# wavey-ai/mel-spec

Hardware: AMD Instinct MI355X
Metric: mel frames/sec/GPU (Whisper 400/160/80 @16 kHz); realtime x vs CPU ref (higher is better)
Workload: dtype f32

## Files before the change

mel_spec_amd/csrc/device_fft.hpp:

```cpp
#pragma once

#if defined(__HIPCC__)
#define MS_DEV __device__ __forceinline__
#ifndef MS_SCHED_LOADS_FIRST
#define MS_SCHED_LOADS_FIRST 0x108
#endif
#define MS_HD __host__ __device__ __forceinline__
#else
#define MS_DEV inline
#define MS_HD inline
#endif
#define MS_RESTRICT __restrict__

namespace melspec {

template <class T>
struct cpx {
    T re, im;
};
using cf = cpx<float>;
using cd = cpx<double>;
struct alignas(8) f2 {
    float x, y;
};
struct alignas(16) f4 {
    float x, y, z, w;
};
struct alignas(16) d2 {
    double x, y;
};

MS_DEV f2 ld2(const float *p) {
#if defined(__HIPCC__)
    typedef float v2f __attribute__((ext_vector_type(2)));
    const v2f v = *reinterpret_cast<const v2f *>(p);
    return f2{v.x, v.y};
#else
    return f2{p[0], p[1]};
#endif
}
MS_DEV f2 ld2_single(const float *p) {
#if defined(__HIPCC__)
    typedef float v2f __attribute__((ext_vector_type(2)));
    typedef const volatile __attribute__((address_space(3))) v2f *lds_ptr;
    const v2f v = *(lds_ptr)(p);
    return f2{v.x, v.y};
#else
    return f2{p[0], p[1]};
#endif
}
MS_DEV f4 ld4(const float *p) {
#if defined(__HIPCC__)
    typedef float v4f __attribute__((ext_vector_type(4)));
    const v4f v = *reinterpret_cast<const v4f *>(p);
    return f4{v.x, v.y, v.z, v.w};
#else
    return f4{p[0], p[1], p[2], p[3]};
#endif
}

template <class T> struct PairOf;
template <> struct PairOf<float> { using type = f2; };
template <> struct PairOf<double> { using type = d2; };
template <class T> MS_DEV cpx<T> ldc(const T *p) {
    const typename PairOf<T>::type v = *reinterpret_cast<const typename PairOf<T>::type *>(p);
    return {v.x, v.y};
}
template <class T> MS_DEV void stc(T *p, cpx<T> v) {
    *reinterpret_cast<typename PairOf<T>::type *>(p) = typename PairOf<T>::type{v.re, v.im};
}

MS_HD float f32_mul_rn(float a, float b) {
#if defined(__HIP_DEVICE_COMPILE__)
    float p = a * b;
    asm("" : "+v"(p));
    return p;
#else
    volatile float p = a * b;
    return p;
#endif
}
MS_DEV int fresh_lane_value(int v) {
#if defined(__HIP_DEVICE_COMPILE__)
    asm volatile("" : "+v"(v));
#endif
    return v;
}
MS_HD float f32_div_rn(float a, float b) {
#if defined(__HIP_DEVICE_COMPILE__)
    return __fdiv_rn(a, b);
#else
    return a / b;
#endif
}
template <class T> MS_DEV cpx<T> operator+(cpx<T> a, cpx<T> b) { return {a.re + b.re, a.im + b.im}; }
template <class T> MS_DEV cpx<T> operator-(cpx<T> a, cpx<T> b) { return {a.re - b.re, a.im - b.im}; }
template <class T> MS_DEV cpx<T> cmul(cpx<T> a, cpx<T> b) { return {a.re * b.re - a.im * b.im, a.re * b.im + a.im * b.re}; }
template <class T> MS_DEV cpx<T> mul_neg_i(cpx<T> a) { return {a.im, -a.re}; }

template <class T>
MS_DEV void bf2(cpx<T> &a, cpx<T> &b) {
    const cpx<T> t = a - b;
    a = a + b;
    b = t;
}

template <class T>
MS_DEV void bf4(cpx<T> &x0, cpx<T> &x1, cpx<T> &x2, cpx<T> &x3) {
    const cpx<T> s0 = x0 + x2, s1 = x0 - x2, s2 = x1 + x3, s3 = mul_neg_i(x1 - x3);
    x0 = s0 + s2;
    x1 = s1 + s3;
    x2 = s0 - s2;
    x3 = s1 - s3;
}

template <class T>
MS_DEV void bf5(cpx<T> &x0, cpx<T> &x1, cpx<T> &x2, cpx<T> &x3, cpx<T> &x4) {
    constexpr T c1 = static_cast<T>(0.30901699437494742410);
    constexpr T c2 = static_cast<T>(-0.80901699437494742410);
    constexpr T s1 = static_cast<T>(0.95105651629515357212);
    constexpr T s2 = static_cast<T>(0.58778525229247312917);
    const cpx<T> t1 = x1 + x4, t2 = x2 + x3, t3 = x1 - x4, t4 = x2 - x3;
    const cpx<T> m1 = {x0.re + c1 * t1.re + c2 * t2.re, x0.im + c1 * t1.im + c2 * t2.im};
    const cpx<T> m2 = {x0.re + c2 * t1.re + c1 * t2.re, x0.im + c2 * t1.im + c1 * t2.im};
    const cpx<T> u1 = {s1 * t3.re + s2 * t4.re, s1 * t3.im + s2 * t4.im};
    const cpx<T> u2 = {s2 * t3.re - s1 * t4.re, s2 * t3.im - s1 * t4.im};
    x0 = x0 + t1 + t2;
    x1 = {m1.re + u1.im, m1.im - u1.re};
    x4 = {m1.re - u1.im, m1.im + u1.re};
    x2 = {m2.re + u2.im, m2.im - u2.re};
    x3 = {m2.re - u2.im, m2.im + u2.re};
}

template <class T>
MS_DEV void fft10(cpx<T> (&x)[10]) {
    cpx<T> a[2][5];
#pragma unroll
    for (int n1 = 0; n1 < 2; ++n1)
#pragma unroll
        for (int n2 = 0; n2 < 5; ++n2) a[n1][n2] = x[(5 * n1 + 2 * n2) % 10];
#pragma unroll
    for (int n2 = 0; n2 < 5; ++n2) bf2(a[0][n2], a[1][n2]);
#pragma unroll
    for (int k1 = 0; k1 < 2; ++k1) bf5(a[k1][0], a[k1][1], a[k1][2], a[k1][3], a[k1][4]);
#pragma unroll
    for (int k1 = 0; k1 < 2; ++k1)
#pragma unroll
        for (int k2 = 0; k2 < 5; ++k2) x[(5 * k1 + 6 * k2) % 10] = a[k1][k2];
}

template <class T>
MS_DEV void fft20(cpx<T> (&x)[20]) {
    cpx<T> a[4][5];
#pragma unroll
    for (int n1 = 0; n1 < 4; ++n1)
#pragma unroll
        for (int n2 = 0; n2 < 5; ++n2) a[n1][n2] = x[(5 * n1 + 4 * n2) % 20];
#pragma unroll
    for (int n2 = 0; n2 < 5; ++n2) bf4(a[0][n2], a[1][n2], a[2][n2], a[3][n2]);
#pragma unroll
    for (int k1 = 0; k1 < 4; ++k1) bf5(a[k1][0], a[k1][1], a[k1][2], a[k1][3], a[k1][4]);
#pragma unroll
    for (int k1 = 0; k1 < 4; ++k1)
#pragma unroll
        for (int k2 = 0; k2 < 5; ++k2) x[(5 * k1 + 16 * k2) % 20] = a[k1][k2];
}

template <class T>
MS_DEV void fft8(cpx<T> (&x)[8]) {
    constexpr T r = static_cast<T>(0.70710678118654752440);
#pragma unroll
    for (int n2 = 0; n2 < 4; ++n2) bf2(x[n2], x[n2 + 4]);
    x[5] = {r * (x[5].re + x[5].im), r * (x[5].im - x[5].re)};
    x[6] = mul_neg_i(x[6]);
    x[7] = {r * (x[7].im - x[7].re), -r * (x[7].re + x[7].im)};
    bf4(x[0], x[1], x[2], x[3]);
    bf4(x[4], x[5], x[6], x[7]);
    const cpx<T> y0 = x[0], y1 = x[4], y2 = x[1], y3 = x[5], y4 = x[2], y5 = x[6], y6 = x[3], y7 = x[7];
    x[0] = y0; x[1] = y1; x[2] = y2; x[3] = y3; x[4] = y4; x[5] = y5; x[6] = y6; x[7] = y7;
}

template <class T>
MS_DEV void fft16(cpx<T> (&x)[16]) {
    constexpr T c1 = static_cast<T>(0.92387953251128675613), s1 = static_cast<T>(0.38268343236508977173);
    constexpr T r = static_cast<T>(0.70710678118654752440);
#pragma unroll
    for (int n2 = 0; n2 < 4; ++n2) bf4(x[n2], x[n2 + 4], x[n2 + 8], x[n2 + 12]);
    x[5] = cmul(x[5], cpx<T>{c1, -s1});
    x[6] = cpx<T>{r * (x[6].re + x[6].im), r * (x[6].im - x[6].re)};
    x[7] = cmul(x[7], cpx<T>{s1, -c1});
    x[9] = cpx<T>{r * (x[9].re + x[9].im), r * (x[9].im - x[9].re)};
    x[10] = mul_neg_i(x[10]);
    x[11] = cpx<T>{r * (x[11].im - x[11].re), -r * (x[11].re + x[11].im)};
    x[13] = cmul(x[13], cpx<T>{s1, -c1});
    x[14] = cpx<T>{r * (x[14].im - x[14].re), -r * (x[14].re + x[14].im)};
    x[15] = cmul(x[15], cpx<T>{-c1, s1});
#pragma unroll
    for (int k1 = 0; k1 < 4; ++k1) bf4(x[4 * k1], x[4 * k1 + 1], x[4 * k1 + 2], x[4 * k1 + 3]);
    cpx<T> y[16];
#pragma unroll
    for (int k1 = 0; k1 < 4; ++k1)
#pragma unroll
        for (int k2 = 0; k2 < 4; ++k2) y[k1 + 4 * k2] = x[4 * k1 + k2];
#pragma unroll
    for (int i = 0; i < 16; ++i) x[i] = y[i];
}

}
```

mel_spec_amd/csrc/fast_tables.hpp:

```cpp
#pragma once
#include <cstdint>
#include <cstring>
#include <vector>

#include "tables.hpp"
#include "whisper_fast.hpp"

namespace melspec {

struct FastTables {
    std::vector<float> blob;
    MelSlots slots{};
    int n_mels = 0;
    int nnz = 0;
    bool interval = false;
};

inline bool build_interval_mel(const std::vector<double> &dense, int n_mels, int bins, int bin_limit,
                               std::vector<float> &b, MelSlots &slots, int lanes = 12, double scale = 0.25,
                               int starts_off = FastBlob::kMelStart, int max_slots = kMaxSlots) {
    const int real = lanes - 1;
    std::vector<int> idx(bin_limit, -1);
    for (int k = 0; k < bin_limit; ++k) {
        int lo = -1, hi = -1;
        for (int m = 0; m < n_mels; ++m)
            if (dense[static_cast<size_t>(m) * bins + k] != 0.0) { if (lo < 0) lo = m; hi = m; }
        if (lo < 0) continue;
        if (hi - lo > 1) return false;
        if (hi != lo) { idx[k] = hi; continue; }
        const double *row = &dense[static_cast<size_t>(lo) * bins];
        int peak = 0;
        for (int q = 1; q < bin_limit; ++q) if (row[q] > row[peak]) peak = q;
        idx[k] = (k <= peak) ? lo : lo + 1;
    }
    int last = -1;
    for (int k = 0; k < bin_limit; ++k) {
        if (idx[k] < 0) continue;
        if (idx[k] < last) return false;
        last = idx[k];
    }
    const int n_int = n_mels + 1;
    std::vector<int> first(n_int, 0), cnt(n_int, 0);
    for (int k = 0; k < bin_limit; ++k) {
        if (idx[k] < 0) continue;
        if (cnt[idx[k]] == 0) first[idx[k]] = k;
        else if (first[idx[k]] + cnt[idx[k]] != k) return false;
        ++cnt[idx[k]];
    }
    const int n_slots = (n_int + real - 1) / real;
    if (n_slots > max_slots || n_slots > kSlotCap) return false;
    slots = MelSlots{};
    slots.n_slots = n_slots;
    for (int s = 0; s < n_slots; ++s) {
        int L = 0;
        for (int j = 0; j < lanes; ++j) {
            const int i = s * real + j;
            if (i < n_int && cnt[i] > L) L = cnt[i];
        }
        slots.len[s] = L;
        slots.woff[s] = static_cast<int>(b.size());
        b.resize(b.size() + static_cast<size_t>(L) * lanes * 2, 0.0f);
        for (int j = 0; j < lanes; ++j) {
            const int i = s * real + j;
            int st = 0;
            if (i < n_int && cnt[i] > 0) {
                st = first[i];
                if (st + L > bin_limit) st = bin_limit - L;
                for (int r = 0; r < L; ++r) {
                    const int k = st + r;
                    if (idx[k] != i) continue;
                    const double rise = i < n_mels ? dense[static_cast<size_t>(i) * bins + k] : 0.0;
                    const double fall = i >= 1 ? dense[static_cast<size_t>(i - 1) * bins + k] : 0.0;
                    b[slots.woff[s] + (r * lanes + j) * 2] = static_cast<float>(scale * rise);
                    b[slots.woff[s] + (r * lanes + j) * 2 + 1] = static_cast<float>(scale * fall);
                }
            }
            std::memcpy(&b[starts_off + s * lanes + j], &st, sizeof(int));
        }
    }
    return true;
}

inline bool build_fast_tables(const std::vector<double> &dense, int n_mels, FastTables &out, bool want_interval = false) {
    constexpr int N = 400, M = 200;
    const int n_slots = (n_mels + kMelJobs - 1) / kMelJobs;
    if (n_mels < 1 || n_slots > kMaxSlots) return false;
    std::vector<float> &b = out.blob;
    b.assign(FastBlob::kMelW, 0.0f);
    const std::vector<double> win = hann_window(N);
    for (int t = 0; t < 10; ++t)
        for (int n1 = 0; n1 < 20; ++n1)
            for (int c = 0; c < 2; ++c) b[FastBlob::kWin + t * FastBlob::kWinStride + 2 * n1 + c] = static_cast<float>(win[20 * n1 + 2 * t + c]);
    for (int t = 0; t < 10; ++t)
        for (int k1 = 0; k1 < 20; ++k1) {
            const double a = -2.0 * kPi * ((t * k1) % M) / M;
            b[FastBlob::kTw1 + t * FastBlob::kTw1Stride + 2 * k1] = static_cast<float>(std::cos(a));
            b[FastBlob::kTw1 + t * FastBlob::kTw1Stride + 2 * k1 + 1] = static_cast<float>(std::sin(a));
        }
    for (int n2 = 0; n2 < 10; ++n2) {
        const double a = -2.0 * kPi * n2 / 10.0;
        b[FastBlob::kMod + 2 * n2] = static_cast<float>(std::cos(a));
        b[FastBlob::kMod + 2 * n2 + 1] = static_cast<float>(std::sin(a));
    }
    for (int j = 0; j < kMelJobs; ++j)
        for (int q = 0; q < 10; ++q) {
            const double a = -2.0 * kPi * (j + 20 * q) / N;
            b[FastBlob::kTw2 + j * 20 + 2 * q] = static_cast<float>(std::cos(a));
            b[FastBlob::kTw2 + j * 20 + 2 * q + 1] = static_cast<float>(std::sin(a));
        }
    const int bins = N / 2 + 1;
    const BandedFilterbank fb = band_filterbank(dense, n_mels, bins, M);
    out.nnz = fb.nnz;
    out.n_mels = n_mels;
    out.interval = false;
    if (want_interval && build_interval_mel(dense, n_mels, bins, M, b, out.slots)) {
        out.interval = true;
        while (b.size() % 4) b.push_back(0.0f);
        return true;
    }
    b.resize(FastBlob::kMelW);
    out.slots = MelSlots{};
    out.slots.n_slots = n_slots;
    for (int i = 0; i < n_slots; ++i) {
        int L = 0;
        for (int j = 0; j < kMelJobs; ++j) {
            const int m = i * kMelJobs + j;
            if (m < n_mels && fb.len[m] > L) L = fb.len[m];
        }
        out.slots.len[i] = L;
        out.slots.woff[i] = static_cast<int>(b.size());
        b.resize(b.size() + static_cast<size_t>(L) * kMelJobs, 0.0f);
        for (int j = 0; j < kMelJobs; ++j) {
            const int m = i * kMelJobs + j;
            int st = 0;
            if (m < n_mels && fb.len[m] > 0) {
                st = fb.start[m];
                if (st + L > M) st = M - L;
                for (int r = 0; r < L; ++r)
                    b[out.slots.woff[i] + r * kMelJobs + j] =
                        static_cast<float>(dense[static_cast<size_t>(m) * bins + st + r]);
            }
            std::memcpy(&b[FastBlob::kMelStart + i * kMelJobs + j], &st, sizeof(int));
        }
    }
    while (b.size() % 4) b.push_back(0.0f);
    return true;
}

inline bool build_fast_tables(double sr, int n_mels, FastTables &out, bool want_interval = false) {
    return build_fast_tables(mel_filterbank(sr, 400, n_mels, -1.0, -1.0, false, true), n_mels, out, want_interval);
}

}

#include "whisper_wave_f64.hpp"
#include "whisper_six.hpp"
#include "whisper_six64.hpp"

namespace melspec {

inline bool build_six_tables(const std::vector<double> &dense, int n_mels, FastTables &out, int max_slots = kSixMaxSlots) {
    constexpr int N = 400, M = 200;
    if (n_mels < 1 || n_mels > kSixOwn * max_slots - 1) return false;
    std::vector<float> &b = out.blob;
    b.assign((SixBlob::kMelStart + max_slots * kSixLanes + 3) & ~3, 0.0f);
    const std::vector<double> win = hann_window(N);
    for (int t = 0; t < 10; ++t)
        for (int n1 = 0; n1 < 20; ++n1)
            for (int c = 0; c < 2; ++c) b[SixBlob::kWin + t * SixBlob::kWinStride + 2 * n1 + c] = static_cast<float>(win[20 * n1 + 2 * t + c]);
    for (int t = 0; t < 10; ++t)
        for (int k1 = 0; k1 < 20; ++k1) {
            const double a = -2.0 * kPi * ((t * k1) % M) / M;
            b[SixBlob::kTw1 + t * SixBlob::kTw1Stride + 2 * k1] = static_cast<float>(std::cos(a));
            b[SixBlob::kTw1 + t * SixBlob::kTw1Stride + 2 * k1 + 1] = static_cast<float>(std::sin(a));
        }
    for (int j = 0; j < kSixLanes; ++j)
        for (int s = 0; s < 11; ++s) {
            int k = j + 20 * s;
            if (j == 0) k = s < 6 ? 20 * s : 10 + 20 * (s - 6);
            const double a = -2.0 * kPi * k / N;
            b[SixBlob::kTw2 + j * SixBlob::kTw2Stride + 2 * s] = static_cast<float>(std::cos(a));
            b[SixBlob::kTw2 + j * SixBlob::kTw2Stride + 2 * s + 1] = static_cast<float>(std::sin(a));
        }
    const int bins = N / 2 + 1;
    out.n_mels = n_mels;
    out.nnz = 0;
    out.interval = build_interval_mel(dense, n_mels, bins, M, b, out.slots, kSixLanes, 0.25, SixBlob::kMelStart, max_slots);
    while (b.size() % 4) b.push_back(0.0f);
    return out.interval;
}

inline bool build_six_tables(double sr, int n_mels, FastTables &out) {
    return build_six_tables(mel_filterbank(sr, 400, n_mels, -1.0, -1.0, false, true), n_mels, out);
}

struct PreciseTables {
    std::vector<uint32_t> blob;
    int mel_off_words = 0;
};

inline bool build_precise_tables(const FastTables &ft, PreciseTables &out, bool power_split) {
    if (!ft.interval) return false;
    constexpr int N = 400, M = 200;
    std::vector<double> t(PreciseBlob::kCount, 0.0);
    const std::vector<double> win = hann_window(N);
    for (int i = 0; i < N; ++i) t[PreciseBlob::kWin + i] = win[i];
    for (int tt = 0; tt < 10; ++tt)
        for (int k1 = 0; k1 < 20; ++k1) {
            const double a = -2.0 * kPi * ((tt * k1) % M) / M;
            t[PreciseBlob::kTw1 + tt * PreciseBlob::kTw1Stride + 2 * k1] = std::cos(a);
            t[PreciseBlob::kTw1 + tt * PreciseBlob::kTw1Stride + 2 * k1 + 1] = std::sin(a);
        }
    for (int n2 = 0; n2 < 10; ++n2) {
        const double a = -2.0 * kPi * n2 / 10.0;
        t[PreciseBlob::kMod + 2 * n2] = std::cos(a);
        t[PreciseBlob::kMod + 2 * n2 + 1] = std::sin(a);
    }
    for (int j = 0; j < kMelJobs; ++j)
        for (int q = 0; q < 10; ++q) {
            const double a = -2.0 * kPi * (j + 20 * q) / N;
            t[PreciseBlob::kTw2 + j * PreciseBlob::kTw2Stride + 2 * q] = power_split ? 2.0 * std::sin(a) : std::cos(a);
            t[PreciseBlob::kTw2 + j * PreciseBlob::kTw2Stride + 2 * q + 1] = power_split ? 4.0 * std::cos(a) : std::sin(a);
        }
    const size_t t_words = t.size() * 2;
    const size_t mel_floats = ft.blob.size() - FastBlob::kMelStart;
    out.mel_off_words = static_cast<int>(t_words);
    out.blob.assign(t_words + mel_floats, 0u);
    std::memcpy(out.blob.data(), t.data(), t.size() * sizeof(double));
    std::memcpy(out.blob.data() + t_words, ft.blob.data() + FastBlob::kMelStart, mel_floats * sizeof(float));
    while (out.blob.size() % 4) out.blob.push_back(0u);
    return true;
}

struct Six64Tables {
    std::vector<uint32_t> blob;
    int mel_off_words = 0;
};

inline bool build_six64_tables(const FastTables &ft6, Six64Tables &out) {
    if (!ft6.interval) return false;
    constexpr int N = 400, M = 200;
    std::vector<double> t(Six64Blob::kCount, 0.0);
    const std::vector<double> win = hann_window(N);
    for (int tt = 0; tt < 10; ++tt)
        for (int n1 = 0; n1 < 20; ++n1)
            for (int c = 0; c < 2; ++c) t[Six64Blob::kWin + tt * Six64Blob::kWinStride + 2 * n1 + c] = win[20 * n1 + 2 * tt + c];
    for (int tt = 0; tt < 10; ++tt)
        for (int k1 = 0; k1 < 20; ++k1) {
            const double a = -2.0 * kPi * ((tt * k1) % M) / M;
            t[Six64Blob::kTw1 + tt * Six64Blob::kTw1Stride + 2 * k1] = std::cos(a);
            t[Six64Blob::kTw1 + tt * Six64Blob::kTw1Stride + 2 * k1 + 1] = std::sin(a);
        }
    for (int j = 0; j < kSixLanes; ++j)
        for (int s = 0; s < 11; ++s) {
            int k = j + 20 * s;
            if (j == 0) k = s < 6 ? 20 * s : 10 + 20 * (s - 6);
            const double a = -2.0 * kPi * k / N;
            t[Six64Blob::kTw2 + j * Six64Blob::kTw2Stride + 2 * s] = 2.0 * std::sin(a);
            t[Six64Blob::kTw2 + j * Six64Blob::kTw2Stride + 2 * s + 1] = 4.0 * std::cos(a);
        }
    const size_t t_words = t.size() * 2;
    const size_t mel_floats = ft6.blob.size() - SixBlob::kMelStart;
    out.mel_off_words = static_cast<int>(t_words);
    out.blob.assign(t_words + mel_floats, 0u);
    std::memcpy(out.blob.data(), t.data(), t.size() * sizeof(double));
    std::memcpy(out.blob.data() + t_words, ft6.blob.data() + SixBlob::kMelStart, mel_floats * sizeof(float));
    while (out.blob.size() % 4) out.blob.push_back(0u);
    return true;
}

}
```

mel_spec_amd/csrc/whisper_six.hpp:

```cpp
#pragma once
#include "whisper_wave.hpp"

namespace melspec {

constexpr int kSixFrames = 6;
constexpr int kSixLanes = 10;
constexpr int kSixOwn = 9;
#ifndef MELSPEC_SIX_WAVES
#define MELSPEC_SIX_WAVES 16
#endif
constexpr int kSixWaves = MELSPEC_SIX_WAVES;
constexpr int kSixMaxSlots = 9;
constexpr int kSixWideSlots = 15;
constexpr int kSixWideWaves = 12;

struct SixBlob {
    static constexpr int kWinStride = 44;
    static constexpr int kWin = 0;
    static constexpr int kTw1 = 10 * kWinStride;
    static constexpr int kTw1Stride = 44;
    static constexpr int kTw2Stride = 28;
    static constexpr int kTw2 = kTw1 + 10 * kTw1Stride;
    static constexpr int kMelStart = kTw2 + 10 * kTw2Stride;
    static constexpr int kMelW = (kMelStart + kSixMaxSlots * kSixLanes + 3) & ~3;
};

struct SixLayout {
    static constexpr int kXRow = 20;
    static constexpr int kXStride = 404;
    static constexpr int kPStride = 213;
    static constexpr int kPmaxOff = 1280;
    static constexpr int kPmaxStride = 12;
    static constexpr int slice_floats() { return kSixFrames * kXStride; }
    MS_HD static constexpr int row_pos(int k1) {
        constexpr int t[20] = {14, 1, 13, 4, 16, 3, 17, 11, 6, 8, 19, 9, 7, 15, 18, 5, 2, 12, 0, 10};
        return t[k1];
    }
    MS_HD static void row_offsets(int j, int &uoff, int &voff) {
        uoff = 0; voff = 0;
        for (int k = 0; k < kSixLanes; ++k)
            if (k == j) { uoff = row_pos(k) * kXRow; voff = row_pos(k == 0 ? 10 : 20 - k) * kXRow; }
    }
};

template <int MELS, int... L>
struct LensSixStatic {
    static constexpr bool kStatic = true;
    static constexpr int kSlots = sizeof...(L);
    static constexpr int kMels = MELS;
    MS_HD static constexpr int len(int i) {
        constexpr int t[sizeof...(L)] = {L...};
        return t[i];
    }
    MS_HD static constexpr int woff(int i) {
        constexpr int t[sizeof...(L)] = {L...};
        int s = 0;
        for (int k = 0; k < i; ++k) s += t[k];
        return SixBlob::kMelW + 2 * kSixLanes * s;
    }
};
using LensSix80 = LensSixStatic<80, 1, 1, 1, 2, 2, 3, 4, 6, 7>;
template <int MELS, int... L>
struct LensSixWideStatic {
    static constexpr bool kStatic = true;
    static constexpr int kSlots = sizeof...(L);
    static constexpr int kMels = MELS;
    static constexpr int kMelW = (SixBlob::kMelStart + kSixWideSlots * kSixLanes + 3) & ~3;
    MS_HD static constexpr int len(int i) {
        constexpr int t[sizeof...(L)] = {L...};
        return t[i];
    }
    MS_HD static constexpr int woff(int i) {
        constexpr int t[sizeof...(L)] = {L...};
        int s = 0;
        for (int k = 0; k < i; ++k) s += t[k];
        return kMelW + 2 * kSixLanes * s;
    }
};
using LensSix128 = LensSixWideStatic<128, 1, 1, 1, 1, 1, 1, 1, 2, 2, 2, 3, 3, 4, 5, 5>;
using LensSix64 = LensSixStatic<64, 2, 2, 2, 3, 4, 6, 10, 10>;
using LensSix40 = LensSixStatic<40, 2, 3, 5, 11, 14>;

template <class In>
MS_DEV void six_phase1(int fl, int t, bool active, int hop, const float *blob, const In *gsrc ,
                       float *slice) {
    if (!active) return;
    const In *s = gsrc + fl * hop + 2 * t;
    cf x[20];
    const float *w = blob + SixBlob::kWin + t * SixBlob::kWinStride;
    f2 sv[20];
#pragma unroll
    for (int n1 = 0; n1 < 20; ++n1) sv[n1] = load2_unaligned(s + 20 * n1);
#if defined(__HIP_DEVICE_COMPILE__)
    __builtin_amdgcn_sched_barrier(MS_SCHED_LOADS_FIRST);
#endif
#pragma unroll
    for (int n1 = 0; n1 < 20; n1 += 2) {
        const f4 wv = ld4(w + 2 * n1);
        x[n1] = {sv[n1].x * wv.x, sv[n1].y * wv.y};
        x[n1 + 1] = {sv[n1 + 1].x * wv.z, sv[n1 + 1].y * wv.w};
    }
    fft20(x);
    const float *tw = blob + SixBlob::kTw1 + t * SixBlob::kTw1Stride;
    float *xo = slice + fl * SixLayout::kXStride + 2 * t;
    *reinterpret_cast<f2 *>(xo + SixLayout::row_pos(0) * SixLayout::kXRow) = f2{x[0].re, x[0].im};
#pragma unroll
    for (int k1 = 1; k1 < 20; ++k1) {
        const f2 wv = *reinterpret_cast<const f2 *>(tw + 2 * k1);
        const cf y = cmul(x[k1], cf{wv.x, wv.y});
        *reinterpret_cast<f2 *>(xo + SixLayout::row_pos(k1) * SixLayout::kXRow) = f2{y.re, y.im};
    }
}

MS_DEV void six_phase2(int fl, int j, bool active, const float *blob, float *slice, int uoff, int voff) {
    if (!active) return;
    const float *ua = slice + fl * SixLayout::kXStride + uoff;
    const float *va = slice + fl * SixLayout::kXStride + voff;
    cf u[10], v[10];
#pragma unroll
    for (int i = 0; i < 5; ++i) {
        const f4 a = *reinterpret_cast<const f4 *>(ua + 4 * i);
        const f4 b = *reinterpret_cast<const f4 *>(va + 4 * i);
        u[2 * i] = {a.x, a.y};
        u[2 * i + 1] = {a.z, a.w};
        v[2 * i] = {b.x, b.y};
        v[2 * i + 1] = {b.z, b.w};
    }
    fft10(u);
    fft10(v);
    const bool lane0 = j == 0;
    const int koff = lane0 ? -110 : j;
    const float *tw = blob + SixBlob::kTw2 + j * SixBlob::kTw2Stride;
    float *p = slice + fl * SixLayout::kPStride;
    auto pair = [&](cf zk, cf zm, cf W, float &pk, float &pm) {
        const cf S = {zk.re + zm.re, zk.im - zm.im};
        const cf D = {zk.re - zm.re, zk.im + zm.im};
        const cf wd = cmul(W, D);
        const float ar = S.re + wd.im, ai = S.im - wd.re;
        const float br = S.re - wd.im, bi = S.im + wd.re;
        pk = ar * ar + ai * ai;
        pm = br * br + bi * bi;
    };
#pragma unroll
    for (int s = 0; s < 10; s += 2) {
        const f4 w2 = *reinterpret_cast<const f4 *>(tw + 2 * s);
        float pk[2], pm[2];
#pragma unroll
        for (int h = 0; h < 2; ++h) {
            const int ss = s + h;
            cf zk, zm;
            if (ss < 6) {
                const cf own = u[(10 - ss) % 10];
                zk = u[ss];
                zm = {lane0 ? own.re : v[9 - ss].re, lane0 ? own.im : v[9 - ss].im};
            } else {
                zk = {lane0 ? v[ss - 6].re : u[ss].re, lane0 ? v[ss - 6].im : u[ss].im};
                zm = {lane0 ? v[15 - ss].re : v[9 - ss].re, lane0 ? v[15 - ss].im : v[9 - ss].im};
            }
            const cf W = h == 0 ? cf{w2.x, w2.y} : cf{w2.z, w2.w};
            pair(zk, zm, W, pk[h], pm[h]);
        }
        const int k = (s < 6 ? j : koff) + 20 * s;
        p[k] = pk[0];
        p[k + 20] = pk[1];
        p[200 - k] = pm[0];
        p[180 - k] = pm[1];
    }
    if (lane0) {
        const f2 w2 = *reinterpret_cast<const f2 *>(tw + 20);
        float pk, pm;
        pair(v[4], v[5], cf{w2.x, w2.y}, pk, pm);
        p[90] = pk;
        p[110] = pm;
    }
}

template <int NSLOTS, class Lens>
MS_DEV void six_phase3_sums(int fl, int j, bool active, const MelSlots &ms, const float *blob, const float *slice,
                            const int (&st)[NSLOTS], float (&rise)[NSLOTS], float (&fprev)[NSLOTS]) {
    const float *p = slice + (active ? fl : 0) * SixLayout::kPStride;
#pragma unroll
    for (int i = 0; i < NSLOTS; ++i) {
        float ar = 0.0f, af = 0.0f;
        if (Lens::kStatic) {
            if (i < Lens::kSlots) {
                const float *pp = p + st[i];
                const float *w = blob + Lens::woff(i < Lens::kSlots ? i : 0) + 2 * j;
#pragma unroll
                for (int r = 0; r < Lens::len(i < Lens::kSlots ? i : 0); ++r) {
                    const f2 wv = ld2_single(w + 2 * kSixLanes * r);
                    const float pv = pp[r];
                    if (r == 0) { ar = wv.x * pv; af = wv.y * pv; }
                    else { ar += wv.x * pv; af += wv.y * pv; }
#if defined(__HIP_DEVICE_COMPILE__)
                    if (Lens::len(i < Lens::kSlots ? i : 0) > 7 && r % 5 == 4 && r + 1 < Lens::len(i < Lens::kSlots ? i : 0))
                        __builtin_amdgcn_sched_barrier(0);
#endif
                }
            }
        } else if (i < ms.n_slots) {
            const float *pp = p + st[i];
            const float *w = blob + ms.woff[i] + 2 * j;
            interval_bins_runtime<2 * kSixLanes>(pp, w, ms.len[i], ar, af);
        }
        rise[i] = ar;
        fprev[i] = af;
    }
}

MS_DEV int six_bits(float v) { return __builtin_bit_cast(int, v); }
MS_DEV float six_float(int v) { return __builtin_bit_cast(float, v); }
MS_DEV int six_imax(int a, int b) { return a > b ? a : b; }
MS_DEV int six_imin(int a, int b) { return a < b ? a : b; }
template <int NSLOTS>
MS_DEV void six_phase3_finish(int fl, int j, bool active, int n_mels, const float (&rise)[NSLOTS],
                              const float (&fnext)[NSLOTS] , float *slice, float (&vals)[NSLOTS]) {
    if (!active) return;
    int mx = 0;
#pragma unroll
    for (int i = 0; i < NSLOTS; ++i) {
        const float e = rise[i] + fnext[i];
        const float v = __builtin_fmaxf(fast_log2(e) * 0.30102999566398120f + 16.0f, 6.0f);
        vals[i] = v;
        if (j < kSixOwn && j + kSixOwn * i < n_mels) mx = six_imax(mx, six_bits(v));
    }
    reinterpret_cast<int *>(slice)[SixLayout::kPmaxOff + fl * SixLayout::kPmaxStride + j] = mx;
}

struct alignas(16) SixI4 { int x, y, z, w; };
struct alignas(8) SixI2 { int x, y; };
MS_DEV float six_out(int c) { return six_float(c) * 0.25f - 3.0f; }
template <int NSLOTS, bool LAYOUT = false, bool GUARD = false, bool KEYS = false, class Out = float>
MS_DEV bool six_phase4(int fl, int j, bool store, bool valid, int n_mels, const float *slice, const float (&vals)[NSLOTS],
                       Out *out_tile, long long row_w, int *kmin = nullptr, int *kmax = nullptr) {
    if (!LAYOUT) { valid = true; row_w = 0; }
    if (!store || j >= kSixOwn) return false;
    int lo = 0;
    if (valid) {
        const int *pm = reinterpret_cast<const int *>(slice) + SixLayout::kPmaxOff + fl * SixLayout::kPmaxStride;
        const SixI4 a = *reinterpret_cast<const SixI4 *>(pm), b = *reinterpret_cast<const SixI4 *>(pm + 4);
        const SixI2 c = *reinterpret_cast<const SixI2 *>(pm + 8);
        const int m0 = six_imax(six_imax(a.x, a.y), six_imax(a.z, a.w));
        const int m1 = six_imax(six_imax(b.x, b.y), six_imax(b.z, b.w));
        lo = six_bits(six_float(six_imax(six_imax(m0, m1), six_imax(c.x, c.y))) - 8.0f);
    }
    Out *o = row_w ? out_tile + static_cast<long long>(j) * row_w + fl : out_tile + static_cast<long long>(fl) * n_mels + j;
    const long long step = row_w ? kSixOwn * row_w : kSixOwn;
    int cmin = 0x7f000000, cmax = 0;
#pragma unroll
    for (int i = 0; i < NSLOTS; ++i) {
        const int m = j + kSixOwn * i;
        if (m < n_mels) {
            const int c = valid ? six_imax(six_bits(vals[i]), lo) : 0x41400000;
            o[i * step] = static_cast<Out>(six_out(c));
            if (GUARD || KEYS) cmin = six_imin(cmin, c);
            if (KEYS) cmax = six_imax(cmax, c);
        }
    }
    if (KEYS) { *kmin = cmin; *kmax = cmax; }
    return GUARD && valid && six_float(cmin) < six_float(lo) + kGuardBand;
}

}
```

Baseline: 3.404 billion.

## Special-case DC/Nyquist bins, FMA-based radix-5 butterfly, and unconditional mel log

Adds a float-specialised radix-5 butterfly that forms the conjugate-pair outputs with FMAs, deriving x4 and x3 from x1 and x2 as 2*m - x. Reworks the real-FFT post-processing so lane 0 handles the DC and Nyquist bins with a closed-form power computation instead of an extra twiddle pair, and shrinks the twiddle table from 11 to 10 entries. The log/max step in phase 3 now runs on all lanes and only the store is predicated, which removes a divergent early return. The risk is small rounding differences from the FMA reassociation, plus wasted work on inactive lanes.

Result: no change. 3.418 billion, median of 6 (+0.4%).

```diff
diff --git a/mel_spec_amd/csrc/device_fft.hpp b/mel_spec_amd/csrc/device_fft.hpp
--- a/mel_spec_amd/csrc/device_fft.hpp
+++ b/mel_spec_amd/csrc/device_fft.hpp
@@ -131,6 +131,18 @@
     x2 = {m2.re + u2.im, m2.im - u2.re};
     x3 = {m2.re - u2.im, m2.im + u2.re};
 }
+MS_DEV void bf5(cf &x0, cf &x1, cf &x2, cf &x3, cf &x4) {
+    constexpr float c1 = 0.30901699437494742410f, c2 = -0.80901699437494742410f;
+    constexpr float s1 = 0.95105651629515357212f, s2 = 0.58778525229247312917f;
+    const cf t1 = x1 + x4, t2 = x2 + x3, t3 = x1 - x4, t4 = x2 - x3;
+    const cf m1 = {x0.re + c1 * t1.re + c2 * t2.re, x0.im + c1 * t1.im + c2 * t2.im};
+    const cf m2 = {x0.re + c2 * t1.re + c1 * t2.re, x0.im + c2 * t1.im + c1 * t2.im};
+    x0 = x0 + t1 + t2;
+    x1 = {__builtin_fmaf(s1, t3.im, __builtin_fmaf(s2, t4.im, m1.re)), __builtin_fmaf(-s1, t3.re, __builtin_fmaf(-s2, t4.re, m1.im))};
+    x2 = {__builtin_fmaf(s2, t3.im, __builtin_fmaf(-s1, t4.im, m2.re)), __builtin_fmaf(-s2, t3.re, __builtin_fmaf(s1, t4.re, m2.im))};
+    x4 = {__builtin_fmaf(2.0f, m1.re, -x1.re), __builtin_fmaf(2.0f, m1.im, -x1.im)};
+    x3 = {__builtin_fmaf(2.0f, m2.re, -x2.re), __builtin_fmaf(2.0f, m2.im, -x2.im)};
+}
 
 template <class T>
 MS_DEV void fft10(cpx<T> (&x)[10]) {
diff --git a/mel_spec_amd/csrc/fast_tables.hpp b/mel_spec_amd/csrc/fast_tables.hpp
--- a/mel_spec_amd/csrc/fast_tables.hpp
+++ b/mel_spec_amd/csrc/fast_tables.hpp
@@ -175,9 +175,9 @@
             b[SixBlob::kTw1 + t * SixBlob::kTw1Stride + 2 * k1 + 1] = static_cast<float>(std::sin(a));
         }
     for (int j = 0; j < kSixLanes; ++j)
-        for (int s = 0; s < 11; ++s) {
+        for (int s = 0; s < 10; ++s) {
             int k = j + 20 * s;
-            if (j == 0) k = s < 6 ? 20 * s : 10 + 20 * (s - 6);
+            if (j == 0) k = s < 5 ? 10 + 20 * s : 20 * s;
             const double a = -2.0 * kPi * k / N;
             b[SixBlob::kTw2 + j * SixBlob::kTw2Stride + 2 * s] = static_cast<float>(std::cos(a));
             b[SixBlob::kTw2 + j * SixBlob::kTw2Stride + 2 * s + 1] = static_cast<float>(std::sin(a));
diff --git a/mel_spec_amd/csrc/whisper_six.hpp b/mel_spec_amd/csrc/whisper_six.hpp
--- a/mel_spec_amd/csrc/whisper_six.hpp
+++ b/mel_spec_amd/csrc/whisper_six.hpp
@@ -129,7 +129,7 @@
     fft10(u);
     fft10(v);
     const bool lane0 = j == 0;
-    const int koff = lane0 ? -110 : j;
+    const int koff = lane0 ? 10 : j;
     const float *tw = blob + SixBlob::kTw2 + j * SixBlob::kTw2Stride;
     float *p = slice + fl * SixLayout::kPStride;
     auto pair = [&](cf zk, cf zm, cf W, float &pk, float &pm) {
@@ -145,33 +145,31 @@
     for (int s = 0; s < 10; s += 2) {
         const f4 w2 = *reinterpret_cast<const f4 *>(tw + 2 * s);
         float pk[2], pm[2];
+        int k[2];
 #pragma unroll
         for (int h = 0; h < 2; ++h) {
             const int ss = s + h;
             cf zk, zm;
-            if (ss < 6) {
-                const cf own = u[(10 - ss) % 10];
+            if (ss < 5) {
+                zk = {lane0 ? v[ss].re : u[ss].re, lane0 ? v[ss].im : u[ss].im};
+                zm = v[9 - ss];
+            } else {
                 zk = u[ss];
-                zm = {lane0 ? own.re : v[9 - ss].re, lane0 ? own.im : v[9 - ss].im};
-            } else {
-                zk = {lane0 ? v[ss - 6].re : u[ss].re, lane0 ? v[ss - 6].im : u[ss].im};
-                zm = {lane0 ? v[15 - ss].re : v[9 - ss].re, lane0 ? v[15 - ss].im : v[9 - ss].im};
+                zm = {lane0 ? u[10 - ss].re : v[9 - ss].re, lane0 ? u[10 - ss].im : v[9 - ss].im};
             }
             const cf W = h == 0 ? cf{w2.x, w2.y} : cf{w2.z, w2.w};
             pair(zk, zm, W, pk[h], pm[h]);
+            k[h] = (ss < 5 ? koff : j) + 20 * ss;
         }
-        const int k = (s < 6 ? j : koff) + 20 * s;
-        p[k] = pk[0];
-        p[k + 20] = pk[1];
-        p[200 - k] = pm[0];
-        p[180 - k] = pm[1];
+        p[k[0]] = pk[0];
+        p[k[1]] = pk[1];
+        p[200 - k[0]] = pm[0];
+        p[200 - k[1]] = pm[1];
     }
     if (lane0) {
-        const f2 w2 = *reinterpret_cast<const f2 *>(tw + 20);
-        float pk, pm;
-        pair(v[4], v[5], cf{w2.x, w2.y}, pk, pm);
-        p[90] = pk;
-        p[110] = pm;
+        const float a = u[0].re + u[0].im, b = u[0].re - u[0].im;
+        p[0] = 4.0f * (a * a);
+        p[200] = 4.0f * (b * b);
     }
 }
 
@@ -215,7 +213,6 @@
 template <int NSLOTS>
 MS_DEV void six_phase3_finish(int fl, int j, bool active, int n_mels, const float (&rise)[NSLOTS],
                               const float (&fnext)[NSLOTS] , float *slice, float (&vals)[NSLOTS]) {
-    if (!active) return;
     int mx = 0;
 #pragma unroll
     for (int i = 0; i < NSLOTS; ++i) {
@@ -224,7 +221,7 @@
         vals[i] = v;
         if (j < kSixOwn && j + kSixOwn * i < n_mels) mx = six_imax(mx, six_bits(v));
     }
-    reinterpret_cast<int *>(slice)[SixLayout::kPmaxOff + fl * SixLayout::kPmaxStride + j] = mx;
+    if (active) reinterpret_cast<int *>(slice)[SixLayout::kPmaxOff + fl * SixLayout::kPmaxStride + j] = mx;
 }
 
 struct alignas(16) SixI4 { int x, y, z, w; };
```
